# alexandrainst/coral

Hardware: AMD Instinct MI355X
Metric: audio-seconds/sec (CTC finetune step: fwd+bwd+allreduce+clip+AdamW), wav2vec2-large, 10 s utterances (higher is better)
Workload: dtype bf16; 1 GPU; wav2vec2-large (XLS-R shape d=1920 L=48 ffn=7680) CTC finetune, 8 x 10 s per GPU, SpecAugment on, activation_dropout 0.1, layerdrop 0 (multi-GPU rule), fp32 master + AdamW + clip 1.0; global_batch=8, frames_per_utt=499, parallelism=dp1

## Files before the change

### coral_amd/csrc/gemm.hip

```cpp
#include "gemm_common.h"
#include <cstdlib>
#include <vector>

struct ProfRec {
  hipEvent_t e0, e1;
  double flops;
  int variant;
};
static bool g_prof_on = false;
static std::vector<ProfRec> g_prof;
hipEvent_t g_gemm_prof_e0 = nullptr, g_gemm_prof_e1 = nullptr;

extern "C" int ca_prof_begin(void) {
  g_prof.clear();
  g_prof_on = true;
  return CA_OK;
}
extern "C" int ca_prof_end(double* ms, int64_t* count, double* flops) {
  g_prof_on = false;
  for (int v = 0; v < 24; ++v) {
    ms[v] = 0.0;
    count[v] = 0;
    flops[v] = 0.0;
  }
  for (auto& r : g_prof) {
    float t = 0.f;
    if (hipEventSynchronize(r.e1) != hipSuccess || hipEventElapsedTime(&t, r.e0, r.e1) != hipSuccess) {
      ca_set_error("ca_prof_end: event query failed");
      return CA_ERR_LAUNCH;
    }
    ms[r.variant] += t;
    count[r.variant] += 1;
    flops[r.variant] += r.flops;
    hipEventDestroy(r.e0);
    hipEventDestroy(r.e1);
  }
  g_prof.clear();
  return CA_OK;
}

extern "C" int ca_gemm_debug_general_epilogue(int on) {
  const int v = on ? 1 : 0;
  for (auto set : {gemm_set_epi_general_s, gemm_set_epi_general_l, gemm_set_epi_general_x, gemm_set_epi_general_fp8})
    if (set(v) != hipSuccess) {
      ca_set_error("ca_gemm_debug_general_epilogue: setting the switch failed");
      return CA_ERR_LAUNCH;
    }
  return CA_OK;
}
static int g_compute_cus = 0;
extern "C" int ca_gemm_set_compute_cus(int n) {
  g_compute_cus = n > 0 ? n : 0;
  return CA_OK;
}
extern "C" int ca_background_update_fits(int32_t* regs) {
  hipFuncAttributes ax, aw;
  const hipError_t e1 = hipFuncGetAttributes(&ax, gemm_x_nt_kernel());
  const hipError_t e2 = hipFuncGetAttributes(&aw, ca_adamw_background_kernel());
  if (e1 != hipSuccess || e2 != hipSuccess) {
    ca_set_error("ca_background_update_fits: hipFuncGetAttributes: %s", hipGetErrorString(e1 != hipSuccess ? e1 : e2));
    return CA_ERR_LAUNCH;
  }
  if (regs) {
    regs[0] = ax.numRegs;
    regs[1] = aw.numRegs;
  }
  const int gx = (ax.numRegs + 7) / 8 * 8, gw = (aw.numRegs + 7) / 8 * 8;
  return 2 * gx + gw <= 512 ? 1 : 0;
}
static unsigned x_device_cus() {
  static const unsigned ncu = [] {
    int dev = 0, n = 256;
    if (hipGetDevice(&dev) == hipSuccess) hipDeviceGetAttribute(&n, hipDeviceAttributeMultiprocessorCount, dev);
    return (unsigned)(n >= 8 ? (n / 8) * 8 : 8);
  }();
  return ncu;
}
static int g_force_kernel = 0;
extern "C" int ca_gemm_force_kernel(int which) {
  g_force_kernel = which;
  return CA_OK;
}
static GemmKnobs gemm_knobs() {
  static const GemmKnobs env = [] {
    GemmKnobs k;
    const auto read = [](const char* name, int& v) { if (const char* e = getenv(name)) v = atoi(e); };
    read("CA_X_PERSIST", k.x_persist);
    read("CA_SKINNY_MB1", k.skinny_mb1);
    read("CA_SKINNY_MB1_ROWS", k.skinny_mb1_rows);
    read("CA_SKINNY_NT", k.skinny_nt);
    read("CA_SKINNY_U", k.skinny_u);
    read("CA_GEMM_PREFER_L", k.prefer_l);
    read("CA_GEMM_L_OVER_X", k.l_over_x);
    read("CA_GEMM_L_MIN", k.l_min);
    read("CA_GEMM_M", k.m_max);
    return k;
  }();
  GemmKnobs k = env;
  k.force_kernel = g_force_kernel;
  k.compute_cus = g_compute_cus;
  k.device_cus = x_device_cus();
  return k;
}
static int ca_gemm_launch(const CaGemmDesc* desc, void* stream);
static int g_last_kind = 0;

extern "C" int ca_gemm_bf16(const CaGemmDesc* desc, void* stream) {
  if (!g_prof_on || desc == nullptr) return ca_gemm_launch(desc, stream);
  ProfRec r;
  hipEventCreate(&r.e0);
  hipEventCreate(&r.e1);
  r.flops = 2.0 * desc->M * (double)desc->N * desc->K * desc->batch1 * desc->batch2;
  g_gemm_prof_e0 = r.e0;
  g_gemm_prof_e1 = r.e1;
  const int rc = ca_gemm_launch(desc, stream);
  g_gemm_prof_e0 = g_gemm_prof_e1 = nullptr;
  r.variant = g_last_kind * 8 + ((desc->a_kseg > 0 || desc->b_kseg > 0) ? 4 : 0) + (desc->a_layout ? 2 : 0) +
              (desc->b_layout ? 1 : 0);
  g_prof.push_back(r);
  return rc;
}

static int gemm_launch_plan(const GemmPlan& p, const CaGemmDesc& d, CaGemmGroup* grp, hipStream_t s, const char* who) {
  if (p.fp8) return gemm_launch_fp8(p, d, s, who);
  switch (p.family) {
    case GEMM_SKINNY: return gemm_launch_skinny(p, d, s, who);
    case GEMM_X: {
      CaGemmGroup one;
      if (!grp) one.d[0] = d, one.count = 0, one.first[0] = 0, one.total = 0;
      return gemm_launch_x(p, grp ? *grp : one, s, who);
    }
    case GEMM_L: return gemm_launch_l(p, d, s, who);
    default: return gemm_launch_s(p, d, s, who);
  }
}

static int gemm_validate_fp8(const CaGemmDesc& d) {
  CA_CHECK_ARG(d.A && d.B && (d.C || d.C2) && d.M > 0 && d.N > 0 && d.K > 0, "ca_gemm_fp8: bad argument");
  CA_CHECK_ARG(d.C8 == nullptr || ((d.epilogue == CA_EPI_GELU || d.epilogue == CA_EPI_DGELU) && d.c8_scale != nullptr && (d.ldc % 8) == 0 &&
                                   ((uintptr_t)d.C8 % 8) == 0),
               "ca_gemm_fp8: C8 needs CA_EPI_GELU / CA_EPI_DGELU, a scale and 8-byte aligned rows");
  CA_CHECK_ARG(d.a_layout == CA_KMAJOR && d.b_layout == CA_KMAJOR && d.batch1 == 1 && d.batch2 == 1 && d.a_kseg == 0 &&
                   d.b_kseg == 0 && !d.a_colsum && !d.c_row_index,
               "ca_gemm_fp8: K-major operands, un-batched, plain rows only");
  CA_CHECK_ARG((d.K % 16) == 0 && (d.lda % 16) == 0 && (d.ldb % 16) == 0 && ((uintptr_t)d.A % 16) == 0 &&
                   ((uintptr_t)d.B % 16) == 0,
               "ca_gemm_fp8: K, lda, ldb must be multiples of 16 bytes and the operands 16-byte aligned");
  return CA_OK;
}
extern "C" int ca_gemm_fp8(const CaGemmDesc* desc, void* stream) {
  CA_CHECK_ARG(desc != nullptr, "ca_gemm_fp8: null descriptor");
  const int rc = gemm_validate_fp8(*desc);
  if (rc != CA_OK) return rc;
  return gemm_launch_plan(gemm_plan_fp8(*desc, gemm_knobs()), *desc, nullptr, (hipStream_t)stream, "ca_gemm_fp8");
}

static int gemm_validate_group(const CaGemmDesc* descs, int32_t count) {
  CA_CHECK_ARG(descs && count >= 1 && count <= X_GROUP_MAX, "ca_gemm_bf16_group: 1..8 problems");
  for (int i = 0; i < count; ++i) {
    const CaGemmDesc* p = descs + i;
    CA_CHECK_ARG(p->A && p->B && p->C && p->M > 0 && p->N > 0 && p->K >= 64, "ca_gemm_bf16_group: bad problem %d", i);
    CA_CHECK_ARG(p->batch1 == 1 && p->batch2 == 1 && p->a_kseg == 0 && p->b_kseg == 0 && p->epilogue == CA_EPI_NONE &&
                     p->bias == nullptr && p->dropout_p == 0.f,
                 "ca_gemm_bf16_group: only plain un-batched problems");
    CA_CHECK_ARG((p->lda % 8) == 0 && (p->ldb % 8) == 0 && ((uintptr_t)p->A % 16) == 0 && ((uintptr_t)p->B % 16) == 0,
                 "ca_gemm_bf16_group: alignment");
    CA_CHECK_ARG(p->a_layout == descs->a_layout && p->b_layout == descs->b_layout,
                 "ca_gemm_bf16_group: the problems differ in operand form");
    CA_CHECK_ARG(p->c_sumsq == nullptr || p->epilogue == CA_EPI_NONE, "ca_gemm_bf16_group: c_sumsq needs a plain epilogue");
  }
  return CA_OK;
}
extern "C" int ca_gemm_bf16_group(const CaGemmDesc* descs, int32_t count, void* stream) {
  const int rc = gemm_validate_group(descs, count);
  if (rc != CA_OK) return rc;
  CaGemmGroup g;
  int total = 0;
  for (int i = 0; i < X_GROUP_MAX; ++i) {
    g.d[i] = descs[i < count ? i : 0];
    g.first[i] = total;
    if (i < count) total += gemm_x_tiles(descs[i]);
  }
  g.total = total;
  g.count = count > 1 ? count : 0;
  const GemmPlan p = gemm_plan_group(descs, count, gemm_knobs());
  ProfRec r;
  if (g_prof_on) {
    hipEventCreate(&r.e0);
    hipEventCreate(&r.e1);
    r.flops = 0.0;
    for (int i = 0; i < count; ++i) r.flops += 2.0 * descs[i].M * (double)descs[i].N * descs[i].K;
    r.variant = p.kind * 8 + p.lay;
    g_gemm_prof_e0 = r.e0;
    g_gemm_prof_e1 = r.e1;
  }
  const int lrc = gemm_launch_plan(p, descs[0], &g, (hipStream_t)stream, "ca_gemm_bf16_group");
  if (g_prof_on) {
    g_gemm_prof_e0 = g_gemm_prof_e1 = nullptr;
    g_prof.push_back(r);
  }
  return lrc;
}

static int gemm_validate_bf16(const CaGemmDesc& d) {
  CA_CHECK_ARG(d.A && d.B &&
                   (d.C || ((d.epilogue == CA_EPI_GELU || d.epilogue == CA_EPI_GELU_RESIDUAL) && d.C2)),
               "ca_gemm_bf16: null operand");
  CA_CHECK_ARG(d.M > 0 && d.N > 0 && d.K > 0, "ca_gemm_bf16: bad shape %d %d %d", d.M, d.N,
               d.K);
  CA_CHECK_ARG(d.batch1 > 0 && d.batch2 > 0, "ca_gemm_bf16: bad batch");
  CA_CHECK_ARG((d.lda % 8) == 0 && (d.ldb % 8) == 0, "ca_gemm_bf16: lda/ldb must be multiples of 8");
  CA_CHECK_ARG((d.sA1 % 8) == 0 && (d.sA2 % 8) == 0 && (d.sB1 % 8) == 0 && (d.sB2 % 8) == 0,
               "ca_gemm_bf16: batch strides must be multiples of 8");
  CA_CHECK_ARG(((uintptr_t)d.A % 16) == 0 && ((uintptr_t)d.B % 16) == 0,
               "ca_gemm_bf16: A/B must be 16-byte aligned");
  CA_CHECK_ARG(d.a_kseg >= 0 && d.b_kseg >= 0, "ca_gemm_bf16: negative kseg");
  if (d.epilogue == CA_EPI_RESIDUAL || d.epilogue == CA_EPI_DGELU || d.epilogue == CA_EPI_GELU_RESIDUAL)
    CA_CHECK_ARG(d.R != nullptr, "ca_gemm_bf16: epilogue needs R");
  CA_CHECK_ARG(d.dropout_p >= 0.f && d.dropout_p < 1.f, "ca_gemm_bf16: bad dropout_p");
  CA_CHECK_ARG(d.C8 == nullptr || ((d.epilogue == CA_EPI_GELU || d.epilogue == CA_EPI_DGELU) && d.c8_scale != nullptr && d.batch1 == 1 && d.batch2 == 1 &&
                                   (d.ldc % 8) == 0 && ((uintptr_t)d.C8 % 8) == 0 && d.M > 32),
               "ca_gemm_bf16: C8 needs CA_EPI_GELU / CA_EPI_DGELU, a scale, an un-batched problem and 8-byte aligned rows");
  if (d.a_colsum)
    CA_CHECK_ARG(d.a_layout == CA_MNMAJOR && d.b_layout == CA_MNMAJOR && d.batch1 == 1 && d.batch2 == 1 && d.a_kseg == 0,
                 "ca_gemm_bf16: a_colsum needs the un-batched weight-gradient form");
  if (d.c_sumsq)
    CA_CHECK_ARG(d.epilogue == CA_EPI_NONE && d.batch1 == 1 && d.batch2 == 1 && d.c_row_index == nullptr && d.c_split_n == 0,
                 "ca_gemm_bf16: c_sumsq needs an un-batched output with the plain epilogue");
  CA_CHECK_ARG(d.a_layout == CA_KMAJOR || d.a_layout == CA_MNMAJOR, "ca_gemm_bf16: bad a_layout");
  CA_CHECK_ARG(d.b_layout == CA_KMAJOR || d.b_layout == CA_MNMAJOR, "ca_gemm_bf16: bad b_layout");
  return CA_OK;
}
static int gemm_validate_skinny(const CaGemmDesc& d) {
  CA_CHECK_ARG(d.c_split_n == 0 || (d.C_hi && (d.c_split_n % 16) == 0 && d.c_split_n < d.N && d.epilogue == CA_EPI_NONE),
               "ca_gemm_bf16: c_split_n needs C_hi, a multiple of 16 below N and no epilogue");
  if (d.a_ln_gamma)
    CA_CHECK_ARG(d.a_ln_beta && d.K <= 2048 && ((uintptr_t)d.a_ln_gamma % 16) == 0 && ((uintptr_t)d.a_ln_beta % 16) == 0,
                 "ca_gemm_bf16: a_ln_gamma needs a_ln_beta, K <= 2048 and 16-byte aligned vectors");
  return CA_OK;
}

static int ca_gemm_launch(const CaGemmDesc* desc, void* stream) {
  CA_CHECK_ARG(desc != nullptr, "ca_gemm_bf16: null descriptor");
  const GemmKnobs knobs = gemm_knobs();
  CaGemmDesc d = *desc;
  d.xcd_balanced = knobs.compute_cus > 0 ? 1 : 0;
  int rc = gemm_validate_bf16(d);
  if (rc != CA_OK) return rc;
  const GemmPlan p = gemm_plan_bf16(d, knobs);
  CA_CHECK_ARG(p.error != GEMM_PLAN_LN_NOT_SKINNY,
               "ca_gemm_bf16: a_ln_gamma exists in the skinny form only (M <= 128, K-major operands, un-batched)");
  CA_CHECK_ARG(p.error != GEMM_PLAN_ROWS_NOT_SKINNY,
               "ca_gemm_bf16: c_row_index / c_split_n exist in the skinny form only (M <= 128, K-major operands, un-batched)");
  g_last_kind = p.kind;
  if (p.family == GEMM_SKINNY && (rc = gemm_validate_skinny(d)) != CA_OK) return rc;
  return gemm_launch_plan(p, d, nullptr, (hipStream_t)stream, "ca_gemm_bf16");
}
```

### coral_amd/csrc/gemm_common.h

```cpp
#pragma once
#include "common.h"
#include "gemm_plan.h"
#include <hip/hip_ext.h>
#include <atomic>
#include <type_traits>

#define TILE_BYTES (BM * BK * 2)
#define XTILE (XBM * BK * 2)

inline __device__ __attribute__((aligned(16))) uint32_t g_ca_zero_page[4];
inline __device__ int g_ca_epi_general = 0;

typedef const __attribute__((address_space(1))) void* gptr_t;
typedef __attribute__((address_space(3))) void* lptr_t;

__device__ __forceinline__ void glds16(const void* g, char* lds_wave_base) {
  asm volatile("s_mov_b32 m0, %1\n\ts_nop 0\n\tglobal_load_lds_dwordx4 %0, off"
               :
               : "v"(g), "s"((uint32_t)(uintptr_t)(lptr_t)lds_wave_base)
               : "memory", "m0");
}

template <int NI, int PC, bool KS = true>
struct MNMajorLoader {
// ... 459 lines not shown
        *(f32x4_t*)(C + 4) = (f32x4_t){v[4], v[5], v[6], v[7]};
#pragma unroll
        for (int e = 0; e < 8; ++e) ssq = fmaf(v[e], v[e], ssq);
      } else {
#pragma unroll
        for (int e = 0; e < 8; ++e)
          if (e < nvalid) {
            const float t = d.accumulate ? C[e] + v[e] : v[e];
            C[e] = t;
            ssq = fmaf(t, t, ssq);
          }
      }
    } else if (d.C) {
      unsigned short* C = (unsigned short*)d.C + coff;
      if (full) {
        if (d.accumulate) {
          const u16x8_t c = *(const u16x8_t*)C;
#pragma unroll
          for (int e = 0; e < 8; ++e) v[e] += bf2f(c[e]);
        }
        u16x8_t o;
#pragma unroll
        for (int e = 0; e < 8; ++e) o[e] = f2bf(v[e]);
        *(u16x8_t*)C = o;
        if (d.c_sumsq != nullptr) {
#pragma unroll
          for (int e = 0; e < 8; ++e) ssq = fmaf(bf2f(o[e]), bf2f(o[e]), ssq);
        }
      } else {
#pragma unroll
        for (int e = 0; e < 8; ++e)
          if (e < nvalid) {
            const unsigned short t = f2bf(d.accumulate ? bf2f(C[e]) + v[e] : v[e]);
            C[e] = t;
            ssq = fmaf(bf2f(t), bf2f(t), ssq);
          }
      }
    }
    if (has_gelu && d.C2) {
      unsigned short* C2 = (unsigned short*)d.C2 + coff;
      if (full) {
        u16x8_t o;
#pragma unroll
        for (int e = 0; e < 8; ++e) o[e] = f2bf(v2[e]);
        *(u16x8_t*)C2 = o;
      } else {
#pragma unroll
        for (int e = 0; e < 8; ++e)
          if (e < nvalid) C2[e] = f2bf(v2[e]);
      }
    }
    if (c8_on) {
      unsigned char* C8 = (unsigned char*)d.C8 + coff;
      float w8[8];
#pragma unroll
      for (int e = 0; e < 8; ++e) w8[e] = epi == CA_EPI_GELU ? v2[e] : v[e];
      if (full) {
        ca_store_fp8x8(C8, w8, s8, amx);
      } else {
#pragma unroll
        for (int e = 0; e < 8; ++e)
          if (e < nvalid) {
            amx = fmaxf(amx, fabsf(w8[e]));
            const float t = fminf(fmaxf(w8[e] * s8, -448.0f), 448.0f);
            C8[e] = (unsigned char)(__builtin_amdgcn_cvt_pk_fp8_f32(t, 0.f, 0u, false) & 0xffu);
          }
      }
    }
  }
  }
  if (d.c_sumsq != nullptr) {
#pragma unroll
    for (int o = 32; o > 0; o >>= 1) ssq += __shfl_xor(ssq, o, 64);
    if (lane == 0 && mw < M && nw < N) d.c_sumsq[(int64_t)(mw >> 6) * ((N + 63) >> 6) + (nw >> 6)] = ssq;
  }
  if (c8_on && d.c8_amax != nullptr) {
#pragma unroll
    for (int o = 32; o > 0; o >>= 1) amx = fmaxf(amx, __shfl_xor(amx, o, 64));
    if (lane == 0 && amx > 0.f)
      atomicMax((unsigned int*)d.c8_amax + (((mw >> 6) * 7 + (nw >> 6)) & (CA_FP8_AMAX_SLOTS - 1)), __float_as_uint(amx));
  }
}

#define X_GROUP_MAX 8
struct CaGemmGroup {
  CaGemmDesc d[X_GROUP_MAX];
  int first[X_GROUP_MAX];
  int count;
  int total;
  int vgrid;
  unsigned* cnt;
  int dyn_first;
};

typedef void (*DescKernel)(const CaGemmDesc);
typedef void (*GroupKernel)(const CaGemmGroup);
int gemm_launch_s(const GemmPlan& p, const CaGemmDesc& d, hipStream_t s, const char* who);
int gemm_launch_l(const GemmPlan& p, const CaGemmDesc& d, hipStream_t s, const char* who);
int gemm_launch_x(const GemmPlan& p, CaGemmGroup& g, hipStream_t s, const char* who);
int gemm_launch_skinny(const GemmPlan& p, const CaGemmDesc& d, hipStream_t s, const char* who);
int gemm_launch_fp8(const GemmPlan& p, const CaGemmDesc& d, hipStream_t s, const char* who);
hipError_t gemm_set_epi_general_s(int on);
hipError_t gemm_set_epi_general_l(int on);
hipError_t gemm_set_epi_general_x(int on);
hipError_t gemm_set_epi_general_fp8(int on);
inline hipError_t gemm_run_epi_general_setter(void (*kernel)(int), int on) {
  hipLaunchKernelGGL(kernel, dim3(1), dim3(1), 0, 0, on);
  const hipError_t e = hipGetLastError();
  return e != hipSuccess ? e : hipDeviceSynchronize();
}
const void* gemm_x_nt_kernel();

extern hipEvent_t g_gemm_prof_e0, g_gemm_prof_e1;
template <class Arg>
int gemm_launch(void (*kernel)(const Arg), dim3 grid, const GemmPlan& p, hipStream_t s, const char* who, const Arg& arg) {
  if (g_gemm_prof_e0)
    hipExtLaunchKernelGGL(kernel, grid, dim3(p.block), p.lds, s, g_gemm_prof_e0, g_gemm_prof_e1, 0, arg);
  else
    hipLaunchKernelGGL(kernel, grid, dim3(p.block), p.lds, s, arg);
  CA_CHECK_LAUNCH(who);
  return CA_OK;
}

template <class T, class KernelOf>
int gemm_allow_lds(std::atomic<uint64_t>& raised, const T* table, int n, KernelOf kernel_of, size_t bytes, const char* who) {
  int dev = 0;
  if (hipGetDevice(&dev) != hipSuccess) dev = 0;
  const uint64_t bit = dev < 64 ? uint64_t(1) << dev : 0;
  if (raised.load(std::memory_order_relaxed) & bit) return CA_OK;
  for (int i = 0; i < n; ++i)
    if (const void* k = kernel_of(table[i])) {
      const hipError_t e = hipFuncSetAttribute(k, hipFuncAttributeMaxDynamicSharedMemorySize, (int)bytes);
      if (e != hipSuccess) {
        ca_set_error("%s: cannot raise the kernel's LDS limit to %zu bytes: %s", who, bytes, hipGetErrorString(e));
        return CA_ERR_LAUNCH;
      }
    }
  raised.fetch_or(bit, std::memory_order_relaxed);
  return CA_OK;
}
template <class K>
int gemm_allow_lds(std::atomic<uint64_t>& raised, K* const* kernels, int n, size_t bytes, const char* who) {
  return gemm_allow_lds(raised, kernels, n, [](K* k) { return (const void*)k; }, bytes, who);
}
```

### coral_amd/csrc/gemm_plan.h

```cpp
#pragma once
#include <stddef.h>
#include <stdint.h>
#include "../../include/coral_amd.h"

#if defined(__HIPCC__)
#define CA_PLAN_FN __host__ __device__ __forceinline__
#else
#define CA_PLAN_FN inline
#endif

#define BM 128
#define BN 128
#define BK 64
#define LBM 256
#define LBN 128
#define XBM 256
#define XBN 256
#define EPI_PITCH 68
#define LDS_BYTES (4 * 64 * EPI_PITCH * 4)
#define M_LDS_BYTES (2 * 4 * BM * BK * 2)
#define L_LDS_BYTES (3 * (LBM + LBN) * BK * 2)
#define X_LDS_BYTES (8 * 64 * EPI_PITCH * 4)
#define X_LAUNCH_LDS (X_LDS_BYTES + 64)
#define SKINNY_LN_PAD 32

CA_PLAN_FN int xcd_split(int ntm, int ntn, int& hb, int& wb) {
  int best = 1, cost = 1 << 30;
#pragma unroll
  for (int bm = 1; bm <= 8; bm *= 2) {
    const int bn = 8 / bm;
    const int c = (ntm + bm - 1) / bm + (ntn + bn - 1) / bn;
    if (c < cost) {
      cost = c;
      best = bm;
    }
  }
  hb = (ntm + best - 1) / best;
  wb = (ntn + 8 / best - 1) / (8 / best);
  return best;
}
CA_PLAN_FN void run_tile(int l, int ntm, int ntn, int& tm, int& tn) {
  if (ntn <= ntm) {
    tm = l / ntn;
    tn = l % ntn;
  } else {
    tn = l / ntm;
    tm = l % ntm;
  }
}
CA_PLAN_FN bool xcd_use_runs(int ntm, int ntn, int hb, int wb, bool bal = false) {
  return bal || 8 * hb * wb * 4 > ntm * ntn * 5;
}
CA_PLAN_FN int xcd_grid(int ntm, int ntn, bool bal = false) {
  if (ntm * ntn <= 8) return ntm * ntn;
  int hb, wb;
  xcd_split(ntm, ntn, hb, wb);
  if (xcd_use_runs(ntm, ntn, hb, wb, bal)) return 8 * ((ntm * ntn + 7) / 8);
  return 8 * hb * wb;
}
CA_PLAN_FN bool xcd_tile(int bid, int ntm, int ntn, int& tm, int& tn, bool bal = false) {
  if (ntm * ntn <= 8) {
    tm = bid / ntn;
    tn = bid % ntn;
    return true;
  }
  int hb, wb;
  const int bm = xcd_split(ntm, ntn, hb, wb);
  const int bn = 8 / bm;
  const int x = bid & 7, idx = bid >> 3;
  if (xcd_use_runs(ntm, ntn, hb, wb, bal)) {
    const int l = x * ((ntm * ntn + 7) / 8) + idx;
    run_tile(l, ntm, ntn, tm, tn);
    return l < ntm * ntn;
  }
  const int bi = x / bn, bj = x % bn;
  tm = bi * hb + idx / wb;
  tn = bj * wb + idx % wb;
  return tm < ntm && tn < ntn;
}
template <int SBM, int SBN>
CA_PLAN_FN bool tile_of_block_g(int bid, int grid, int ntm, int ntn, int& tm, int& tn, bool bal = false) {
  if (grid == xcd_grid(ntm, ntn, bal)) {
    return xcd_tile(bid, ntm, ntn, tm, tn, bal);
  }
  const int x = bid & 7, i = bid >> 3;
  const int per = SBM * SBN;
  const int sb = (i / per) * 8 + x, t = i % per;
  const int nsbn = (ntn + SBN - 1) / SBN;
  const int sbm = sb / nsbn, sbn = sb % nsbn;
  tm = sbm * SBM + (t % SBM);
  tn = sbn * SBN + (t / SBM);
  return tm < ntm && tn < ntn;
}
template <int SBM, int SBN>
CA_PLAN_FN unsigned tile_grid(int ntm, int ntn, bool bal = false) {
  if (ntm * ntn < 4 * 8 * SBM * SBN) return (unsigned)xcd_grid(ntm, ntn, bal);
  const int nsb = ((ntm + SBM - 1) / SBM) * ((ntn + SBN - 1) / SBN);
  return (unsigned)(((nsb + 7) / 8) * 8 * SBM * SBN);
}

struct GemmKnobs {
  int x_persist = 1;
  int skinny_mb1 = 4;
  int skinny_mb1_rows = 16;
  int skinny_nt = 0;
  int skinny_u = 0;
  int prefer_l = 3;
  int l_over_x = 0;
  int l_min = 100;
  int m_max = 256;
  int force_kernel = 0;
  int compute_cus = 0;
  unsigned device_cus = 256;
};
inline unsigned gemm_compute_cus(const GemmKnobs& k) {
  if (k.compute_cus <= 0) return k.device_cus;
  const unsigned c = (unsigned)(k.compute_cus >= 8 ? (k.compute_cus / 8) * 8 : 8);
  return c < k.device_cus ? c : k.device_cus;
}

enum GemmFamily { GEMM_SKINNY = 0, GEMM_S = 1, GEMM_M = 2, GEMM_L = 3, GEMM_X = 4 };
enum GemmPlanError { GEMM_PLAN_OK = 0, GEMM_PLAN_LN_NOT_SKINNY = 1, GEMM_PLAN_ROWS_NOT_SKINNY = 2 };
struct GemmPlan {
  int error = GEMM_PLAN_OK;
  int family = GEMM_S;
  int fp8 = 0;
  int lay = 0;
  int ks = 0;
  int mb = 0, nch = 0, u = 0, nt = 0;
  unsigned grid_x = 1, grid_y = 1, grid_z = 1, block = 256;
  size_t lds = 0;
  unsigned vgrid = 0;
  int persistent = 0, dyn_first = 0;
  int kind = 0;
};
inline int gemm_x_tiles(const CaGemmDesc& d) { return ((d.M + XBM - 1) / XBM) * ((d.N + XBN - 1) / XBN); }

inline void gemm_plan_x_geometry(GemmPlan& p, unsigned vgrid, unsigned nbz, const GemmKnobs& k) {
  const unsigned ncu = gemm_compute_cus(k);
  p.family = GEMM_X;
  p.kind = 2;
  p.vgrid = vgrid;
  p.dyn_first = k.compute_cus > 0 ? 1 : 0;
  p.persistent = (k.x_persist && nbz == 1 && vgrid > ncu) ? 1 : 0;
  p.grid_x = p.persistent ? ncu : vgrid;
  p.grid_z = nbz;
  p.block = 512;
  p.lds = X_LAUNCH_LDS;
}

inline bool gemm_takes_skinny(const CaGemmDesc& d, const GemmKnobs& k) {
  const bool skinny_wide = d.M > 32 && d.M <= 128 && d.C8 == nullptr && d.c_sumsq == nullptr &&
                           (d.a_ln_gamma || d.c_row_index || d.c_split_n > 0 || d.N <= 8192 || d.M <= 64);
  return k.force_kernel == 0 && (d.M <= 32 || skinny_wide) && d.a_layout == CA_KMAJOR && d.b_layout == CA_KMAJOR &&
         d.batch1 == 1 && d.batch2 == 1 && d.a_kseg == 0 && d.b_kseg == 0 && d.dropout_p == 0.f &&
         d.epilogue != CA_EPI_DGELU;
}
inline void gemm_plan_skinny(GemmPlan& p, const CaGemmDesc& d, const GemmKnobs& k) {
  p.family = GEMM_SKINNY;
  p.kind = 0;
  unsigned gy = d.M <= 32 ? 1u : (unsigned)((d.M + 31) / 32);
  const bool rows16 = k.skinny_mb1 && d.M > k.skinny_mb1_rows && d.M > 16 &&
                      (unsigned)((d.N + 15) / 16) * gy <= (unsigned)k.skinny_mb1 * k.device_cus;
  if (rows16) gy = (unsigned)((d.M + 15) / 16);
  int nt = 16;
  if (d.M <= 16 || rows16) {
    const unsigned want = 3u * k.device_cus / 4u;
    if ((unsigned)((d.N + 15) / 16) * gy < want) nt = (unsigned)((d.N + 7) / 8) * gy >= want ? 8 : 4;
    if (k.skinny_nt == 4 || k.skinny_nt == 8 || k.skinny_nt == 16) nt = k.skinny_nt;
  }
  p.grid_x = (unsigned)((d.N + nt - 1) / nt);
  p.grid_y = gy;
  p.block = 256;
  p.mb = (d.M <= 16 || rows16) ? 1 : 2;
  p.nt = nt;
  p.u = 8;
  if (d.a_ln_gamma) {
    p.nch = (d.K + 511) / 512 <= 2 ? 2 : (d.K + 511) / 512;
    p.lds = (size_t)4 * p.mb * 256 * sizeof(float) + (size_t)16 * p.mb * (d.K + SKINNY_LN_PAD) * 2;
    return;
  }
  p.lds = (size_t)4 * p.mb * 256 * sizeof(float);
  if (p.mb == 1) {
    const int per = ((d.K + 31) / 32 + 3) / 4;
    p.u = per <= 8 ? 8 : (per <= 16 ? 16 : 32);
    if (k.skinny_u == 8 || k.skinny_u == 16 || k.skinny_u == 32) p.u = k.skinny_u;
  }
}

inline int gemm_tiled_family(const CaGemmDesc& d, const GemmKnobs& k) {
  const int force = k.force_kernel;
  const int lay = (d.a_layout ? 2 : 0) + (d.b_layout ? 1 : 0);
  const bool ks = d.a_kseg > 0 || d.b_kseg > 0;
  const int64_t nb = (int64_t)d.batch1 * d.batch2;
  const int64_t tiles_l = (int64_t)((d.M + LBM - 1) / LBM) * ((d.N + LBN - 1) / LBN) * nb;
  bool use_l = force == 2 && !ks;
  const int xtm = (d.M + XBM - 1) / XBM, xtn = (d.N + XBN - 1) / XBN;
  const int64_t xt = (int64_t)xtm * xtn * nb;
  const int64_t cus = (int64_t)gemm_compute_cus(k);
  const double xwaves = (double)xt / (double)cus;
  const double xeff = xwaves / (double)((xt + cus - 1) / cus);
  const double xfill = ((double)d.M * d.N) / ((double)xtm * XBM * (double)xtn * XBN);
  const bool tn = d.a_layout == CA_MNMAJOR && d.b_layout == CA_MNMAJOR;
  bool use_x = force == 0 && d.K >= 512 && xt >= 160 && xeff * xfill >= (tn ? 0.60 : 0.70);
  if (force == 3 || d.a_colsum) use_x = true;
  const int lox = k.l_over_x;
  if (k.prefer_l && force == 0 && !ks && d.K >= 512 && tiles_l >= k.l_min &&
      (tiles_l <= cus * k.prefer_l || (use_x && lox)) && !d.a_colsum &&
      (!use_x || (lox == 1 && !tn) || lox == 2 || (lox == 3 && lay == 0))) {
    use_l = true;
    use_x = false;
  }
  const int ntm = (d.M + BM - 1) / BM, ntn = (d.N + BN - 1) / BN;
  const int64_t ts = (int64_t)ntm * ntn;
  if (force == 0 && k.compute_cus > 0 && cus < (int64_t)k.device_cus && nb == 1 && !ks && d.K >= 512 && !d.a_colsum &&
      d.M > 128) {
    auto rounds = [](int64_t tiles, int64_t slots) { return (double)((tiles + slots - 1) / slots); };
    const double cx = rounds(xt, cus) * 4.0, cl = rounds(tiles_l, cus) * 2.0 / (tn ? 0.85 : 0.93),
                 cs = rounds(ts, 2 * cus) * 2.0 / (tn ? 0.6 : 0.8), cm = rounds(ts, cus) * 1.0 / 0.6;
    int family = GEMM_X;
    double best = cx;
    if (cl < best) { best = cl; family = GEMM_L; }
    if (cs < best) { best = cs; family = GEMM_S; }
    if (cm < best) { best = cm; family = GEMM_M; }
    return family;
  }
// ... 74 lines not shown
```

### coral_amd/csrc/gemm_x.hip

```cpp
#include "gemm_common.h"

static_assert(X_LDS_BYTES >= 4 * XTILE, "kernel X: the epilogue staging covers the two stages of both operand tiles");

#define X_CNT_SLOTS 64
__device__ unsigned g_x_cnt[X_CNT_SLOTS][8];
#ifdef X_STAMPS
__device__ long long g_x_stamps[512 * 8 * 8];
extern "C" int ca_gemm_x_stamps(long long* host, int n) {
  return (int)hipMemcpyFromSymbol(host, HIP_SYMBOL(g_x_stamps), (size_t)n * sizeof(long long));
}
#endif
template <int AL, int BL, bool KS>
__device__ __forceinline__ void gemm_x_body(const CaGemmGroup& grp) {
  extern __shared__ __attribute__((aligned(16))) char smem[];
  const int tid = threadIdx.x;
  const int lane = tid & 63;
  const int wave = __builtin_amdgcn_readfirstlane(tid >> 6);
  const int wm = wave >> 2, wn = wave & 3;
  const int vgrid = grp.vgrid;
  const int xcd = (int)blockIdx.x & 7;
  const int npx = ((int)gridDim.x - xcd + 7) >> 3;
  const int nvx = (vgrid - xcd + 7) >> 3;
  const int ndyn = nvx > npx ? nvx - npx : 0;
  volatile unsigned* nextw = (volatile unsigned*)(smem + X_LDS_BYTES);
  KMajorStream<4> la_k, lb_k;
  MNMajorStream<4, 32> la_f, lb_f;
  MNMajorLoader<4, 32, KS> la_m, lb_m;
  int vb = (int)blockIdx.x;
  int dbase = npx, dcount = ndyn;
  if (grp.cnt != nullptr && grp.dyn_first) {
    dbase = 0;
    dcount = nvx;
    if (tid == 0) {
      const unsigned i = __hip_atomic_fetch_add(&grp.cnt[xcd], 1u, __ATOMIC_RELAXED, __HIP_MEMORY_SCOPE_AGENT);
      if (i == (unsigned)(dcount + npx - 1)) __hip_atomic_store(&grp.cnt[xcd], 0u, __ATOMIC_RELAXED, __HIP_MEMORY_SCOPE_AGENT);
      nextw[1] = i;
    }
    __syncthreads();
    const unsigned i = (unsigned)__builtin_amdgcn_readfirstlane((int)nextw[1]);
    vb = i < (unsigned)dcount ? xcd + 8 * (int)i : vgrid;
  }
  for (int iter = 0; vb < vgrid; ++iter) {
  int vb_next = vgrid;
  if (grp.cnt != nullptr && tid == 0) {
    const unsigned i = __hip_atomic_fetch_add(&grp.cnt[xcd], 1u, __ATOMIC_RELAXED, __HIP_MEMORY_SCOPE_AGENT);
    if (i == (unsigned)(dcount + npx - 1)) __hip_atomic_store(&grp.cnt[xcd], 0u, __ATOMIC_RELAXED, __HIP_MEMORY_SCOPE_AGENT);
    nextw[iter & 1] = i;
  }
  bool live = true;
  int which = 0, gt = 0;
  if (grp.count > 1) {
    gt = (vb & 7) * (vgrid >> 3) + (vb >> 3);
    live = gt < grp.total;
    if (live) {
#pragma unroll
      for (int i = 1; i < X_GROUP_MAX; ++i)
        if (grp.count > i && gt >= grp.first[i]) which = i;
    }
  }
  const CaGemmDesc d = grp.d[which];
  int tm = 0, tn = 0;
  if (live) {
    if (grp.count > 1)
      run_tile(gt - grp.first[which], (d.M + XBM - 1) / XBM, (d.N + XBN - 1) / XBN, tm, tn);
    else
      live = tile_of_block_g<4, 8>(vb, vgrid, (d.M + XBM - 1) / XBM, (d.N + XBN - 1) / XBN, tm, tn, d.xcd_balanced != 0);
  }
  if (live) {
  const int m0 = tm * XBM, n0 = tn * XBN;
  const int z = blockIdx.z;
  const int z1 = z / d.batch2, z2 = z % d.batch2;
  const __bf16* A = (const __bf16*)d.A + z1 * d.sA1 + z2 * d.sA2;
  const __bf16* B = (const __bf16*)d.B + z1 * d.sB1 + z2 * d.sB2;

  auto init_loaders = [&](int row0, int col0) {
    if (AL == CA_KMAJOR)
      la_k.init(A, d.lda, row0, d.M, wave, lane);
    else if (KS)
      la_m.init(A, d.lda, d.a_kseg, d.a_kseg_stride, row0, d.M, wave, lane);
    else
      la_f.init(A, d.lda, row0, d.M, wave, lane);
    if (BL == CA_KMAJOR)
      lb_k.init(B, d.ldb, col0, d.N, wave, lane);
    else if (KS)
      lb_m.init(B, d.ldb, d.b_kseg, d.b_kseg_stride, col0, d.N, wave, lane);
    else
      lb_f.init(B, d.ldb, col0, d.N, wave, lane);
  };
  init_loaders(m0, n0);

  f32x4_t acc[8][4];
#pragma unroll
  for (int i = 0; i < 8; ++i)
#pragma unroll
    for (int j = 0; j < 4; ++j) acc[i][j] = (f32x4_t){0.f, 0.f, 0.f, 0.f};
  float xbias[8];
  if constexpr (!KS) epi_load_bias(d, lane, n0 + wn * 64, z1, z2, xbias);
#ifdef X_STAMPS
  long long stamp_dma = 0, stamp_bar = 0;
#endif
  const int cs_parts = ((d.N + XBN - 1) / XBN) < 8 ? ((d.N + XBN - 1) / XBN) : 8;
  const bool do_colsum = d.a_colsum != nullptr && tn < cs_parts;
  float csum0 = 0.f, csum1 = 0.f;

  const int K = d.K;
  const int nk = (K + BK - 1) / BK;

  auto burst = [&](int kt) {
    if (kt >= nk) return;
    char* na = smem + (kt & 1) * XTILE;
    char* nb = na + 2 * XTILE;
    const bool full = (kt + 1) * BK <= K;
    if (full) {
#pragma unroll
      for (int part = 0; part < 4; ++part) {
        if (AL == CA_MNMAJOR && KS)
          la_m.issue_one(na, wave, lane, kt * BK, K, part);
        else if (AL == CA_KMAJOR)
          la_k.issue_one(na, wave, part);
        else
          la_f.issue_one(na, wave, part);
        if (BL == CA_MNMAJOR && KS)
          lb_m.issue_one(nb, wave, lane, kt * BK, K, part);
        else if (BL == CA_KMAJOR)
          lb_k.issue_one(nb, wave, part);
        else
          lb_f.issue_one(nb, wave, part);
      }
    } else {
#pragma unroll
      for (int part = 0; part < 4; ++part) {
        if (AL == CA_MNMAJOR && KS)
          la_m.issue_one(na, wave, lane, kt * BK, K, part);
        else if (AL == CA_KMAJOR)
          la_k.issue_one_tail(na, wave, K - kt * BK, part);
        else
          la_f.issue_one_tail(na, wave, lane, K - kt * BK, part);
        if (BL == CA_MNMAJOR && KS)
          lb_m.issue_one(nb, wave, lane, kt * BK, K, part);
        else if (BL == CA_KMAJOR)
          lb_k.issue_one_tail(nb, wave, K - kt * BK, part);
        else
          lb_f.issue_one_tail(nb, wave, lane, K - kt * BK, part);
      }
    }
    if (AL == CA_KMAJOR) la_k.advance();
    if (AL == CA_MNMAJOR && !KS) la_f.advance();
    if (BL == CA_KMAJOR) lb_k.advance();
    if (BL == CA_MNMAJOR && !KS) lb_f.advance();
  };
  auto zero_tail = [&](int kt) {
    if (kt != nk - 1 || nk * BK == K) return;
// ... 3 lines not shown
    if (AL == CA_KMAJOR) la_k.zero_fix(na, wave, lane, krem);
    if (AL == CA_MNMAJOR && !KS) la_f.zero_fix(na, wave, lane, krem);
    if (BL == CA_KMAJOR) lb_k.zero_fix(nb, wave, lane, krem);
    if (BL == CA_MNMAJOR && !KS) lb_f.zero_fix(nb, wave, lane, krem);
    asm volatile("s_waitcnt lgkmcnt(0)" ::: "memory");
  };
  const uint32_t lds0 = (uint32_t)(uintptr_t)(lptr_t)smem;
  uint32_t abase[8], bbase[4];
  if (AL == CA_KMAJOR) {
    const int r = wm * 128 + (lane & 15);
#pragma unroll
    for (int sh = 0; sh < 2; ++sh) abase[sh] = lds0 + r * 128 + (((4 * sh + (lane >> 4)) ^ ((r >> 1) & 7)) * 16);
  } else {
    const int g = lane >> 4, q = (lane & 15) >> 2, pp = lane & 3;
    const int swz = q | ((g & 1) << 2);
#pragma unroll
    for (int f = 0; f < 8; ++f) {
      const int c = ((((wm * 128 + f * 16) >> 3) + (pp >> 1)) ^ (swz << 1));
      abase[f] = lds0 + (8 * g + q) * 512 + c * 16 + (pp & 1) * 8;
    }
  }
  if (BL == CA_KMAJOR) {
    const int r = wn * 64 + (lane & 15);
#pragma unroll
    for (int sh = 0; sh < 2; ++sh)
      bbase[sh] = lds0 + 2 * XTILE + r * 128 + (((4 * sh + (lane >> 4)) ^ ((r >> 1) & 7)) * 16);
  } else {
    const int g = lane >> 4, q = (lane & 15) >> 2, pp = lane & 3;
    const int swz = q | ((g & 1) << 2);
#pragma unroll
    for (int f = 0; f < 4; ++f) {
      const int c = ((((wn * 64 + f * 16) >> 3) + (pp >> 1)) ^ (swz << 1));
      bbase[f] = lds0 + 2 * XTILE + (8 * g + q) * 512 + c * 16 + (pp & 1) * 8;
    }
  }
  bf16x8_t A0[4], A1[4], B0[4], B1[4];
#define X_RD_A(ST, SH, F, dst)                                                            \
  do {                                                                                    \
    if (AL == CA_KMAJOR)                                                                  \
      dst = lds_read_b128<(ST) * XTILE + (F) * 2048>(abase[SH]);                          \
    else                                                                                  \
      dst = lds_read_tr<(ST) * XTILE + (SH) * 16384, 2048>(abase[F]);                     \
  } while (0)
#define X_RD_B(ST, SH, F, dst)                                                            \
  do {                                                                                    \
    if (BL == CA_KMAJOR)                                                                  \
      dst = lds_read_b128<(ST) * XTILE + (F) * 2048>(bbase[SH]);                          \
    else                                                                                  \
      dst = lds_read_tr<(ST) * XTILE + (SH) * 16384, 2048>(bbase[F]);                     \
  } while (0)
#define X_SB __builtin_amdgcn_sched_barrier(0)
#define X_MM2(IH, AF, BF, I, J)                                                                                   \
  do {                                                                                                            \
    acc[(IH) * 4 + (I)][J] = __builtin_amdgcn_mfma_f32_16x16x32_bf16(BF[J], AF[I], acc[(IH) * 4 + (I)][J], 0, 0, 0); \
    acc[(IH) * 4 + (I)][(J) + 1] =                                                                                \
        __builtin_amdgcn_mfma_f32_16x16x32_bf16(BF[(J) + 1], AF[I], acc[(IH) * 4 + (I)][(J) + 1], 0, 0, 0);       \
    X_SB;                                                                                                         \
  } while (0)
  auto colsum_acc = [&](bool cs_step, int ih, bf16x8_t (&af)[4]) {
    if (AL == CA_MNMAJOR && cs_step) {
      f32x4_t z;
      if (wn == 0)
        z = __builtin_bit_cast(f32x4_t, af[0]);
      else if (wn == 1)
        z = __builtin_bit_cast(f32x4_t, af[1]);
      else if (wn == 2)
        z = __builtin_bit_cast(f32x4_t, af[2]);
      else
        z = __builtin_bit_cast(f32x4_t, af[3]);
      typedef __attribute__((ext_vector_type(2))) __bf16 bf16x2_t;
      const bf16x2_t ones = __builtin_bit_cast(bf16x2_t, 0x3F803F80u);
      float s = ih == 0 ? csum0 : csum1;
#pragma unroll
      for (int q = 0; q < 4; ++q) {
        const unsigned int wq = __float_as_uint(z[q]);
        s = __builtin_amdgcn_fdot2_f32_bf16(__builtin_bit_cast(bf16x2_t, wq), ones, s, false);
      }
      if (ih == 0)
        csum0 = s;
      else
        csum1 = s;
    }
  };
  auto kstep = [&](auto st_c, int kt) {
    constexpr int ST = decltype(st_c)::value;
    const bool cs_step = do_colsum && (kt % cs_parts) == tn;
    constexpr bool LATE_BURST = AL == CA_MNMAJOR && BL == CA_MNMAJOR && !KS;
    if (!LATE_BURST && wave >= 4) burst(kt + 1);
    lds_wait(B0);
    lds_wait(A0);
    colsum_acc(cs_step, 0, A0);
    X_SB;
    __builtin_amdgcn_s_setprio(1);
    X_MM2(0, A0, B0, 0, 0); X_RD_A(ST, 0, 4, A1[0]); X_SB;
    X_MM2(0, A0, B0, 0, 2); X_RD_A(ST, 0, 5, A1[1]); X_SB;
    X_MM2(0, A0, B0, 1, 0); X_RD_A(ST, 0, 6, A1[2]); X_SB;
    X_MM2(0, A0, B0, 1, 2); X_RD_A(ST, 0, 7, A1[3]); X_SB;
    X_MM2(0, A0, B0, 2, 0);
    X_MM2(0, A0, B0, 2, 2);
    X_MM2(0, A0, B0, 3, 0);
    X_MM2(0, A0, B0, 3, 2);
    __builtin_amdgcn_s_setprio(0);
    if (LATE_BURST && wave >= 4) burst(kt + 1);
    lds_wait(A1);
    colsum_acc(cs_step, 1, A1);
    X_SB;
    __builtin_amdgcn_s_setprio(1);
    X_MM2(1, A1, B0, 0, 0); X_RD_B(ST, 1, 0, B1[0]); X_SB;
    X_MM2(1, A1, B0, 0, 2); X_RD_B(ST, 1, 1, B1[1]); X_SB;
    X_MM2(1, A1, B0, 1, 0); X_RD_B(ST, 1, 2, B1[2]); X_SB;
    X_MM2(1, A1, B0, 1, 2); X_RD_B(ST, 1, 3, B1[3]); X_SB;
    X_MM2(1, A1, B0, 2, 0); X_RD_A(ST, 1, 0, A0[0]); X_SB;
    X_MM2(1, A1, B0, 2, 2); X_RD_A(ST, 1, 1, A0[1]); X_SB;
    X_MM2(1, A1, B0, 3, 0); X_RD_A(ST, 1, 2, A0[2]); X_SB;
    X_MM2(1, A1, B0, 3, 2); X_RD_A(ST, 1, 3, A0[3]); X_SB;
    __builtin_amdgcn_s_setprio(0);
    lds_wait(B1);
    lds_wait(A0);
    colsum_acc(cs_step, 0, A0);
    X_SB;
    __builtin_amdgcn_s_setprio(1);
    X_MM2(0, A0, B1, 0, 0); X_RD_A(ST, 1, 4, A1[0]); X_SB;
    X_MM2(0, A0, B1, 0, 2); X_RD_A(ST, 1, 5, A1[1]); X_SB;
    X_MM2(0, A0, B1, 1, 0); X_RD_A(ST, 1, 6, A1[2]); X_SB;
    X_MM2(0, A0, B1, 1, 2); X_RD_A(ST, 1, 7, A1[3]); X_SB;
    X_MM2(0, A0, B1, 2, 0);
    X_MM2(0, A0, B1, 2, 2);
    X_MM2(0, A0, B1, 3, 0);
    X_MM2(0, A0, B1, 3, 2);
    __builtin_amdgcn_s_setprio(0);
    lds_wait(A1);
    colsum_acc(cs_step, 1, A1);
#ifdef X_STAMPS
    const long long st0 = __builtin_amdgcn_s_memtime();
#endif
    asm volatile("s_waitcnt vmcnt(0)" ::: "memory");
#ifdef X_STAMPS
    const long long st1 = __builtin_amdgcn_s_memtime();
#endif
    zero_tail(kt + 1);
    __builtin_amdgcn_s_barrier();
    asm volatile("" ::: "memory");
#ifdef X_STAMPS
    const long long st2 = __builtin_amdgcn_s_memtime();
    stamp_dma += st1 - st0;
    stamp_bar += st2 - st1;
#endif
    if (wave < 4) burst(kt + 2);
    X_SB;
    __builtin_amdgcn_s_setprio(1);
    X_MM2(1, A1, B1, 0, 0); X_RD_B(1 - ST, 0, 0, B0[0]); X_SB;
    X_MM2(1, A1, B1, 0, 2); X_RD_B(1 - ST, 0, 1, B0[1]); X_SB;
    X_MM2(1, A1, B1, 1, 0); X_RD_B(1 - ST, 0, 2, B0[2]); X_SB;
    X_MM2(1, A1, B1, 1, 2); X_RD_B(1 - ST, 0, 3, B0[3]); X_SB;
    X_MM2(1, A1, B1, 2, 0); X_RD_A(1 - ST, 0, 0, A0[0]); X_SB;
    X_MM2(1, A1, B1, 2, 2); X_RD_A(1 - ST, 0, 1, A0[1]); X_SB;
    X_MM2(1, A1, B1, 3, 0); X_RD_A(1 - ST, 0, 2, A0[2]); X_SB;
    X_MM2(1, A1, B1, 3, 2); X_RD_A(1 - ST, 0, 3, A0[3]); X_SB;
    __builtin_amdgcn_s_setprio(0);
  };
#ifdef X_STAMPS
  const long long stamp_t0 = __builtin_amdgcn_s_memtime();
#endif
  burst(0);
  asm volatile("s_waitcnt vmcnt(0) lgkmcnt(0)" ::: "memory");
  zero_tail(0);
  __builtin_amdgcn_s_barrier();
  asm volatile("" ::: "memory");
#ifdef X_STAMPS
  const long long stamp_t1 = __builtin_amdgcn_s_memtime();
  const long long stamp_r1 = __builtin_amdgcn_s_memrealtime();
  __builtin_amdgcn_s_waitcnt(0xC07F);
#endif
  X_RD_B(0, 0, 0, B0[0]); X_RD_B(0, 0, 1, B0[1]); X_RD_B(0, 0, 2, B0[2]); X_RD_B(0, 0, 3, B0[3]);
  X_RD_A(0, 0, 0, A0[0]); X_RD_A(0, 0, 1, A0[1]); X_RD_A(0, 0, 2, A0[2]); X_RD_A(0, 0, 3, A0[3]);
  if (wave < 4) burst(1);
  for (int kt = 0; kt < nk; kt += 2) {
    kstep(std::integral_constant<int, 0>{}, kt);
    if (kt + 1 < nk) kstep(std::integral_constant<int, 1>{}, kt + 1);
  }
#undef X_RD_A
#undef X_RD_B
#undef X_MM2
#undef X_SB
#ifdef X_STAMPS
  const long long stamp_t2 = __builtin_amdgcn_s_memtime();
  const long long stamp_r2 = __builtin_amdgcn_s_memrealtime();
#endif
  if (AL == CA_MNMAJOR && do_colsum) {
#pragma unroll
    for (int ih = 0; ih < 2; ++ih) {
      float s = ih == 0 ? csum0 : csum1;
      s += __shfl_xor(s, 16, 64);
      s += __shfl_xor(s, 32, 64);
      const int m = m0 + wm * 128 + (ih * 4 + wn) * 16 + (lane & 15);
      if (lane < 16 && m < d.M) d.a_colsum[(int64_t)tn * d.a_colsum_ld + m] = s;
    }
  }
  unsigned nxt = 0;
  if (grp.cnt != nullptr) nxt = (unsigned)__builtin_amdgcn_readfirstlane((int)nextw[iter & 1]);
  asm volatile("s_waitcnt lgkmcnt(0)" ::: "memory");
  __builtin_amdgcn_s_barrier();
  asm volatile("" ::: "memory");
  if (grp.cnt != nullptr) vb_next = nxt < (unsigned)dcount ? xcd + 8 * (dbase + (int)nxt) : vgrid;
#pragma unroll
  for (int ih = 0; ih < 2; ++ih) {
    f32x4_t half[4][4];
#pragma unroll
    for (int i = 0; i < 4; ++i)
#pragma unroll
      for (int j = 0; j < 4; ++j) half[i][j] = acc[ih * 4 + i][j];
    gemm_epilogue(d, half, smem, wave, lane, m0 + wm * 128 + ih * 64, n0 + wn * 64, z, z1, z2, KS ? nullptr : &xbias);
    asm volatile("s_waitcnt lgkmcnt(0)" ::: "memory");
  }
  if (grp.cnt != nullptr) __syncthreads();
#ifdef X_STAMPS
  {
    asm volatile("s_waitcnt vmcnt(0)" ::: "memory");
    const long long stamp_t3 = __builtin_amdgcn_s_memtime();
    if (lane == 0 && iter == 0) {
      long long* o = g_x_stamps + ((size_t)blockIdx.x * 8 + wave) * 8;
      o[0] = stamp_t1 - stamp_t0;
      o[1] = stamp_t2 - stamp_t1;
      o[2] = stamp_t3 - stamp_t2;
      o[3] = stamp_dma;
      o[4] = stamp_bar;
      o[5] = nk;
      o[6] = stamp_r2 - stamp_r1;
    }
  }
#endif
  }
  else if (grp.cnt != nullptr) {
    __syncthreads();
    const unsigned i = (unsigned)__builtin_amdgcn_readfirstlane((int)nextw[iter & 1]);
    vb_next = i < (unsigned)dcount ? xcd + 8 * (dbase + (int)i) : vgrid;
  }
  if (grp.cnt == nullptr) break;
  vb = vb_next;
  }
}

template <int AL, int BL, bool KS>
__global__ __launch_bounds__(512) void ca_gemm_kernel_x(const CaGemmGroup grp) {
  gemm_x_body<AL, BL, KS>(grp);
}
template <>
__global__ __launch_bounds__(512) __attribute__((amdgpu_num_vgpr(112)))
void ca_gemm_kernel_x<CA_KMAJOR, CA_KMAJOR, false>(const CaGemmGroup grp) {
  gemm_x_body<CA_KMAJOR, CA_KMAJOR, false>(grp);
}

static const GroupKernel k_gemm_x[8] = {ca_gemm_kernel_x<0, 0, false>, ca_gemm_kernel_x<0, 1, false>, ca_gemm_kernel_x<1, 0, false>,
                                        ca_gemm_kernel_x<1, 1, false>, ca_gemm_kernel_x<0, 0, false>, ca_gemm_kernel_x<0, 1, true>,
                                        ca_gemm_kernel_x<1, 0, true>,  ca_gemm_kernel_x<1, 1, true>};

__global__ void gemm_set_epi_general_x_kernel(int on) { g_ca_epi_general = on; }
hipError_t gemm_set_epi_general_x(int on) { return gemm_run_epi_general_setter(gemm_set_epi_general_x_kernel, on); }
const void* gemm_x_nt_kernel() { return (const void*)ca_gemm_kernel_x<0, 0, false>; }

int gemm_launch_x(const GemmPlan& p, CaGemmGroup& g, hipStream_t s, const char* who) {
  static unsigned seq = 0;
  static std::atomic<uint64_t> raised{0};
  if (int rc = gemm_allow_lds(raised, k_gemm_x, 8, p.lds, who)) return rc;
  g.vgrid = (int)p.vgrid;
  g.cnt = nullptr;
  g.dyn_first = p.dyn_first;
  dim3 grid(p.vgrid, 1, p.grid_z);
  if (p.persistent) {
    unsigned* base = nullptr;
    if (hipGetSymbolAddress((void**)&base, HIP_SYMBOL(g_x_cnt)) == hipSuccess && base) {
      g.cnt = base + (size_t)(seq++ % X_CNT_SLOTS) * 8;
      grid.x = p.grid_x;
    }
  }
  return gemm_launch(k_gemm_x[p.lay + 4 * p.ks], grid, p, s, who, g);
}
#undef X_CNT_SLOTS
```

Baseline: 1109 audio-seconds/sec.

## Schedule half-empty edge tiles separately in grouped X GEMM and idle unused waves

For grouped MN-major X GEMMs, tiles are split into a full-tile list and an edge-tile list, and each XCD gets a balanced share of full tiles with edge tiles filling the rest. In edge tiles where M or N covers at most half the tile, waves whose sub-tile lies outside the matrix skip the MFMA work and the epilogue. They still take part in the DMA bursts and barriers, and can do the column-sum work when that is needed. The wave-to-subtile mapping is remapped for N-half tiles. The aim is to stop wasting compute on padded regions and to even out per-XCD load, at the cost of more complex tile indexing and extra code paths in the kernel.

```diff
diff --git a/coral_amd/csrc/gemm.hip b/coral_amd/csrc/gemm.hip
--- a/coral_amd/csrc/gemm.hip
+++ b/coral_amd/csrc/gemm.hip
@@ -86,6 +86,7 @@
     GemmKnobs k;
     const auto read = [](const char* name, int& v) { if (const char* e = getenv(name)) v = atoi(e); };
     read("CA_X_PERSIST", k.x_persist);
+    read("CA_X_EDGE", k.x_edge);
     read("CA_SKINNY_MB1", k.skinny_mb1);
     read("CA_SKINNY_MB1_ROWS", k.skinny_mb1_rows);
     read("CA_SKINNY_NT", k.skinny_nt);
@@ -127,7 +128,7 @@
     case GEMM_SKINNY: return gemm_launch_skinny(p, d, s, who);
     case GEMM_X: {
       CaGemmGroup one;
-      if (!grp) one.d[0] = d, one.count = 0, one.first[0] = 0, one.total = 0;
+      if (!grp) one.d[0] = d, one.count = 0, one.first[0] = 0, one.total = 0, one.nfull = 0;
       return gemm_launch_x(p, grp ? *grp : one, s, who);
     }
     case GEMM_L: return gemm_launch_l(p, d, s, who);
@@ -175,13 +176,8 @@
   const int rc = gemm_validate_group(descs, count);
   if (rc != CA_OK) return rc;
   CaGemmGroup g;
-  int total = 0;
-  for (int i = 0; i < X_GROUP_MAX; ++i) {
-    g.d[i] = descs[i < count ? i : 0];
-    g.first[i] = total;
-    if (i < count) total += gemm_x_tiles(descs[i]);
-  }
-  g.total = total;
+  for (int i = 0; i < X_GROUP_MAX; ++i) g.d[i] = descs[i < count ? i : 0];
+  x_group_lists(descs, count, g.first, g.ffirst, g.efirst, g.total, g.nfull);
   g.count = count > 1 ? count : 0;
   const GemmPlan p = gemm_plan_group(descs, count, gemm_knobs());
   ProfRec r;
diff --git a/coral_amd/csrc/gemm_common.h b/coral_amd/csrc/gemm_common.h
--- a/coral_amd/csrc/gemm_common.h
+++ b/coral_amd/csrc/gemm_common.h
@@ -565,12 +565,15 @@
   }
 }
 
-#define X_GROUP_MAX 8
 struct CaGemmGroup {
   CaGemmDesc d[X_GROUP_MAX];
   int first[X_GROUP_MAX];
   int count;
   int total;
+  int edge;
+  int nfull;
+  int ffirst[X_GROUP_MAX];
+  int efirst[X_GROUP_MAX];
   int vgrid;
   unsigned* cnt;
   int dyn_first;
diff --git a/coral_amd/csrc/gemm_plan.h b/coral_amd/csrc/gemm_plan.h
--- a/coral_amd/csrc/gemm_plan.h
+++ b/coral_amd/csrc/gemm_plan.h
@@ -101,6 +101,7 @@
 
 struct GemmKnobs {
   int x_persist = 1;
+  int x_edge = 1;
   int skinny_mb1 = 4;
   int skinny_mb1_rows = 16;
   int skinny_nt = 0;
@@ -132,9 +133,62 @@
   size_t lds = 0;
   unsigned vgrid = 0;
   int persistent = 0, dyn_first = 0;
+  int edge = 0;
   int kind = 0;
 };
 inline int gemm_x_tiles(const CaGemmDesc& d) { return ((d.M + XBM - 1) / XBM) * ((d.N + XBN - 1) / XBN); }
+
+CA_PLAN_FN int x_full_dim(int n) { return n / XBM + ((n % XBM) > XBM / 2 ? 1 : 0); }
+CA_PLAN_FN int x_full_tiles(int M, int N) { return x_full_dim(M) * x_full_dim(N); }
+CA_PLAN_FN void x_edge_tile(int e, int ntm, int ntn, int fn, int& tm, int& tn) {
+  const int ncol = fn < ntn ? ntm : 0;
+  if (e < ncol) {
+    tm = e;
+    tn = ntn - 1;
+  } else {
+    tm = ntm - 1;
+    tn = e - ncol;
+  }
+}
+CA_PLAN_FN bool x_group_visit(int vb, int vgrid, int nfull, int total, bool& is_edge, int& idx) {
+  const int x = vb & 7, i = vb >> 3, per = vgrid >> 3;
+  const int f0 = (int)(((int64_t)x * nfull) >> 3), f1 = (int)(((int64_t)(x + 1) * nfull) >> 3);
+  is_edge = i >= f1 - f0;
+  idx = is_edge ? x * per - f1 + i : f0 + i;
+  return !is_edge || idx < total - nfull;
+}
+#define X_GROUP_MAX 8
+inline void x_group_lists(const CaGemmDesc* descs, int count, int (&first)[X_GROUP_MAX], int (&ffirst)[X_GROUP_MAX],
+                          int (&efirst)[X_GROUP_MAX], int& total, int& nfull) {
+  total = nfull = 0;
+  for (int i = 0; i < X_GROUP_MAX; ++i) {
+    first[i] = total;
+    ffirst[i] = nfull;
+    efirst[i] = total - nfull;
+    if (i < count) {
+      total += ((descs[i].M + XBM - 1) / XBM) * ((descs[i].N + XBN - 1) / XBN);
+      nfull += x_full_tiles(descs[i].M, descs[i].N);
+    }
+  }
+}
+template <class Dims>
+CA_PLAN_FN void x_group_tile(bool is_edge, int idx, int count, const int (&ffirst)[X_GROUP_MAX], const int (&efirst)[X_GROUP_MAX],
+                             Dims dims, int& which, int& tm, int& tn) {
+  which = 0;
+  int base = 0;
+#pragma unroll
+  for (int i = 1; i < X_GROUP_MAX; ++i) {
+    const int fi = ffirst[i], ei = efirst[i];
+    const int li = is_edge ? ei : fi;
+    if (count > i && idx >= li) which = i, base = li;
+  }
+  int M, N;
+  dims(which, M, N);
+  if (is_edge)
+    x_edge_tile(idx - base, (M + XBM - 1) / XBM, (N + XBN - 1) / XBN, x_full_dim(N), tm, tn);
+  else
+    run_tile(idx - base, x_full_dim(M), x_full_dim(N), tm, tn);
+}
 
 inline void gemm_plan_x_geometry(GemmPlan& p, unsigned vgrid, unsigned nbz, const GemmKnobs& k) {
   const unsigned ncu = gemm_compute_cus(k);
@@ -142,6 +196,7 @@
   p.kind = 2;
   p.vgrid = vgrid;
   p.dyn_first = k.compute_cus > 0 ? 1 : 0;
+  p.edge = k.x_edge ? 1 : 0;
   p.persistent = (k.x_persist && nbz == 1 && vgrid > ncu) ? 1 : 0;
   p.grid_x = p.persistent ? ncu : vgrid;
   p.grid_z = nbz;
diff --git a/coral_amd/csrc/gemm_x.hip b/coral_amd/csrc/gemm_x.hip
--- a/coral_amd/csrc/gemm_x.hip
+++ b/coral_amd/csrc/gemm_x.hip
@@ -16,7 +16,8 @@
   const int tid = threadIdx.x;
   const int lane = tid & 63;
   const int wave = __builtin_amdgcn_readfirstlane(tid >> 6);
-  const int wm = wave >> 2, wn = wave & 3;
+  const int wm0 = wave >> 2, wn0 = wave & 3;
+  constexpr bool EDGE = AL == CA_MNMAJOR && BL == CA_MNMAJOR && !KS;
   const int vgrid = grp.vgrid;
   const int xcd = (int)blockIdx.x & 7;
   const int npx = ((int)gridDim.x - xcd + 7) >> 3;
@@ -49,25 +50,47 @@
   }
   bool live = true;
   int which = 0, gt = 0;
+  const bool edge_on = EDGE && grp.edge != 0;
+  int tm = 0, tn = 0;
   if (grp.count > 1) {
-    gt = (vb & 7) * (vgrid >> 3) + (vb >> 3);
-    live = gt < grp.total;
-    if (live) {
-#pragma unroll
-      for (int i = 1; i < X_GROUP_MAX; ++i)
-        if (grp.count > i && gt >= grp.first[i]) which = i;
+    if (edge_on) {
+      bool edge_list;
+      live = x_group_visit(vb, vgrid, grp.nfull, grp.total, edge_list, gt);
+      if (live)
+        x_group_tile(edge_list, gt, grp.count, grp.ffirst, grp.efirst,
+                     [&](int i, int& M, int& N) { M = grp.d[i].M, N = grp.d[i].N; }, which, tm, tn);
+    } else {
+      gt = (vb & 7) * (vgrid >> 3) + (vb >> 3);
+      live = gt < grp.total;
+      if (live) {
+#pragma unroll
+        for (int i = 1; i < X_GROUP_MAX; ++i)
+          if (grp.count > i && gt >= grp.first[i]) which = i;
+      }
     }
   }
   const CaGemmDesc d = grp.d[which];
-  int tm = 0, tn = 0;
   if (live) {
-    if (grp.count > 1)
+    if (grp.count > 1 && edge_on)
+      ;
+    else if (grp.count > 1)
       run_tile(gt - grp.first[which], (d.M + XBM - 1) / XBM, (d.N + XBN - 1) / XBN, tm, tn);
     else
       live = tile_of_block_g<4, 8>(vb, vgrid, (d.M + XBM - 1) / XBM, (d.N + XBN - 1) / XBN, tm, tn, d.xcd_balanced != 0);
   }
   if (live) {
   const int m0 = tm * XBM, n0 = tn * XBN;
+  int wm = wm0, wn = wn0;
+  bool busy = true, cs_idle = false;
+  if (edge_on) {
+    const bool m_half = d.M - m0 <= XBM / 2, n_half = d.N - n0 <= XBN / 2;
+    if (n_half) {
+      wm = (wave >> 1) & 1;
+      wn = 2 * (wave >> 2) + (wave & 1);
+    }
+    busy = !(m_half && wm == 1) && !(n_half && wn >= 2);
+    cs_idle = !busy && !(m_half && wm == 1);
+  }
   const int z = blockIdx.z;
   const int z1 = z / d.batch2, z2 = z % d.batch2;
   const __bf16* A = (const __bf16*)d.A + z1 * d.sA1 + z2 * d.sA2;
@@ -237,9 +260,54 @@
         csum1 = s;
     }
   };
+  auto colsum_idle = [&](auto st_c) {
+    constexpr int ST = decltype(st_c)::value;
+    if constexpr (EDGE) {
+      const int g = lane >> 4, q = (lane & 15) >> 2, pp = lane & 3;
+      const int swz = q | ((g & 1) << 2);
+      bf16x8_t fr[4];
+#pragma unroll
+      for (int ih = 0; ih < 2; ++ih) {
+        const int c = ((((wm * 128 + (ih * 4 + wn) * 16) >> 3) + (pp >> 1)) ^ (swz << 1));
+        const uint32_t a = lds0 + (8 * g + q) * 512 + c * 16 + (pp & 1) * 8;
+        fr[ih * 2 + 0] = lds_read_tr<ST * XTILE, 2048>(a);
+        fr[ih * 2 + 1] = lds_read_tr<ST * XTILE + 16384, 2048>(a);
+      }
+      lds_wait(fr);
+      typedef __attribute__((ext_vector_type(2))) __bf16 bf16x2_t;
+      const bf16x2_t ones = __builtin_bit_cast(bf16x2_t, 0x3F803F80u);
+#pragma unroll
+      for (int i = 0; i < 4; ++i) {
+        const f32x4_t z = __builtin_bit_cast(f32x4_t, fr[i]);
+        float s = i < 2 ? csum0 : csum1;
+#pragma unroll
+        for (int q4 = 0; q4 < 4; ++q4) {
+          const unsigned int wq = __float_as_uint(z[q4]);
+          s = __builtin_amdgcn_fdot2_f32_bf16(__builtin_bit_cast(bf16x2_t, wq), ones, s, false);
+        }
+        if (i < 2)
+          csum0 = s;
+        else
+          csum1 = s;
+      }
+    }
+  };
   auto kstep = [&](auto st_c, int kt) {
     constexpr int ST = decltype(st_c)::value;
     const bool cs_step = do_colsum && (kt % cs_parts) == tn;
+    if (EDGE && !busy) {
+      if (wave >= 4) {
+        __builtin_amdgcn_s_sleep(4);
+        burst(kt + 1);
+      }
+      if (cs_idle && cs_step) colsum_idle(st_c);
+      asm volatile("s_waitcnt vmcnt(0)" ::: "memory");
+      zero_tail(kt + 1);
+      __builtin_amdgcn_s_barrier();
+      asm volatile("" ::: "memory");
+      if (wave < 4) burst(kt + 2);
+      return;
+    }
     constexpr bool LATE_BURST = AL == CA_MNMAJOR && BL == CA_MNMAJOR && !KS;
     if (!LATE_BURST && wave >= 4) burst(kt + 1);
     lds_wait(B0);
@@ -327,8 +395,10 @@
   const long long stamp_r1 = __builtin_amdgcn_s_memrealtime();
   __builtin_amdgcn_s_waitcnt(0xC07F);
 #endif
-  X_RD_B(0, 0, 0, B0[0]); X_RD_B(0, 0, 1, B0[1]); X_RD_B(0, 0, 2, B0[2]); X_RD_B(0, 0, 3, B0[3]);
-  X_RD_A(0, 0, 0, A0[0]); X_RD_A(0, 0, 1, A0[1]); X_RD_A(0, 0, 2, A0[2]); X_RD_A(0, 0, 3, A0[3]);
+  if (!EDGE || busy) {
+    X_RD_B(0, 0, 0, B0[0]); X_RD_B(0, 0, 1, B0[1]); X_RD_B(0, 0, 2, B0[2]); X_RD_B(0, 0, 3, B0[3]);
+    X_RD_A(0, 0, 0, A0[0]); X_RD_A(0, 0, 1, A0[1]); X_RD_A(0, 0, 2, A0[2]); X_RD_A(0, 0, 3, A0[3]);
+  }
   if (wave < 4) burst(1);
   for (int kt = 0; kt < nk; kt += 2) {
     kstep(std::integral_constant<int, 0>{}, kt);
@@ -358,6 +428,7 @@
   __builtin_amdgcn_s_barrier();
   asm volatile("" ::: "memory");
   if (grp.cnt != nullptr) vb_next = nxt < (unsigned)dcount ? xcd + 8 * (dbase + (int)nxt) : vgrid;
+  if (!EDGE || busy) {
 #pragma unroll
   for (int ih = 0; ih < 2; ++ih) {
     f32x4_t half[4][4];
@@ -367,6 +438,7 @@
       for (int j = 0; j < 4; ++j) half[i][j] = acc[ih * 4 + i][j];
     gemm_epilogue(d, half, smem, wave, lane, m0 + wm * 128 + ih * 64, n0 + wn * 64, z, z1, z2, KS ? nullptr : &xbias);
     asm volatile("s_waitcnt lgkmcnt(0)" ::: "memory");
+  }
   }
   if (grp.cnt != nullptr) __syncthreads();
 #ifdef X_STAMPS
@@ -421,6 +493,7 @@
   g.vgrid = (int)p.vgrid;
   g.cnt = nullptr;
   g.dyn_first = p.dyn_first;
+  g.edge = p.edge;
   dim3 grid(p.vgrid, 1, p.grid_z);
   if (p.persistent) {
     unsigned* base = nullptr;
```

Result: no change. 1115 audio-seconds/sec (median of 6 runs) (+0.6%).
